# projectchrono/DEM-Engine

Hardware: AMD Instinct MI355X
Metric: clump*steps/s (higher is better)
Workload: dtype f32 physics / f64 geometry

## Files before the change

### dem-engine_amd/csrc/deme_kernels.h

```cpp
#pragma once
#include "deme_device.h"
#include "deme_owner_cols.h"

namespace deme_dev {

#define DEME_NULL_BINID_DEV 0xFFFFFFFFu
#define DEME_ST_VELOCITY 1u
#define DEME_ST_NONFINITE 2u
#define DEME_ST_INCIDENCE 4u
#define DEME_MAX_BINS_PER_SPHERE 0xFFFFFFu

struct DetectCounters {
    unsigned long long nContactsRaw;
    unsigned int nActiveBins;
    unsigned int maxInBin;
    unsigned int status;
    unsigned int pad0;
    unsigned long long nIncidence;
    unsigned int pad[8];
};

#define DEME_KEY_SEGS 64u
#define DEME_KEY_SEG_STRIDE 16u
struct DetectBlock {
    DetectCounters c;
    unsigned long long segCount[DEME_KEY_SEGS];
    unsigned long long segCtr[DEME_KEY_SEGS * DEME_KEY_SEG_STRIDE];
};
struct DetectHead {
    DetectCounters c;
    unsigned long long segCount[DEME_KEY_SEGS];
};
struct KeyArena {
    uint64_t* keys;
    unsigned long long* ctr;
    uint64_t segCap;
    uint32_t segMask;
};
__device__ inline uint32_t arena_seg(const KeyArena& a) {
    return blockIdx.x & a.segMask;
}
__device__ inline unsigned long long arena_reserve(const KeyArena& a, uint32_t seg, unsigned long long n) {
    return atomicAdd(&a.ctr[seg * DEME_KEY_SEG_STRIDE], n);
}
__device__ inline void arena_store(const KeyArena& a, uint32_t seg, unsigned long long slot, uint64_t key) {
    if (slot < a.segCap)
        a.keys[(uint64_t)seg * a.segCap + slot] = key;
}
__device__ void bin_stats_block(const uint2* __restrict__ perBlock, uint32_t nBlocks, uint32_t block, DetectCounters* ctr);
__global__ __launch_bounds__(256) void k_compact_keys(const uint64_t* __restrict__ in, uint64_t segCap, DetectBlock* blk, uint32_t xOff,
                                                      uint64_t* __restrict__ out, const uint2* __restrict__ stats, uint32_t nStats) {
    __shared__ unsigned long long sStart, sCount;
    const uint32_t seg = blockIdx.y;
    if (threadIdx.x < 64) {
        static_assert(DEME_KEY_SEGS == 64, "one lane per segment");
        const unsigned long long raw = blk->segCtr[threadIdx.x * DEME_KEY_SEG_STRIDE];
        if (stats && seg == 0 && blockIdx.x == 0)
            blk->segCount[threadIdx.x] = raw;
        const unsigned long long cnt = min(raw, (unsigned long long)segCap);
        unsigned long long inc = cnt;
        for (int d = 1; d < 64; d <<= 1) {
            const unsigned long long u = __shfl_up(inc, d);
            if ((int)threadIdx.x >= d)
                inc += u;
        }
        if (threadIdx.x == seg)
            sStart = inc - cnt, sCount = cnt;
    }
    __syncthreads();
    const uint64_t i = ((uint64_t)xOff + blockIdx.x) * blockDim.x + threadIdx.x;
    if (i < sCount)
        out[sStart + i] = in[(uint64_t)seg * segCap + i];
    if (stats && seg == 0)
        for (uint32_t b = blockIdx.x; b * 2048u < nStats; b += gridDim.x)
            bin_stats_block(stats, nStats, b, &blk->c);
}

__global__ __launch_bounds__(256) void k_margins(const DevParams p, OwnerRec* owners, uint32_t drift,
                                                 DetectCounters* ctr) {
    const uint32_t o = blockIdx.x * blockDim.x + threadIdx.x;
    if (o >= p.nOwners)
        return;
    OwnerRec* r = owners + o;
    const double vx = r->vx, vy = r->vy, vz = r->vz;
    float absv = (float)sqrt(vx * vx + vy * vy + vz * vz);
    if (!isfinite(absv))
        atomicOr(&ctr->status, DEME_ST_NONFINITE);
    else if (absv > p.errOutVel)
        atomicOr(&ctr->status, DEME_ST_VELOCITY);
    if (absv > p.approxMaxVel)
        absv = p.approxMaxVel;
    const float extra = p.familyTrivial ? 0.f : p.familyExtra[fam_of(r->family)];
    r->margin = (float)((double)(absv * p.expSafetyMulti + p.expSafetyAdder) * (double)p.h * (double)drift + (double)extra);
}

__global__ __launch_bounds__(256) void k_set_margins(uint32_t n, OwnerRec* owners, const float* m, const uint32_t* __restrict__ o2e) {
    const uint32_t o = blockIdx.x * blockDim.x + threadIdx.x;
    if (o < n)
        owners[o].margin = m[o2e ? o2e[o] : o];
}

struct ObjWorld {
    double x, y, z;
    float dx, dy, dz;
    float size1, nsign, margin;
    uint32_t type, family;
};

__global__ __launch_bounds__(256) void k_sphere_prep(const DevParams p, const OwnerRec* __restrict__ owners,
                                                     const SphereRec* __restrict__ spheres, GeoRec* __restrict__ geo,
                                                     uint4* __restrict__ binLo, uint2* __restrict__ binN,
                                                     uint32_t* __restrict__ partial, const KeyArena ar, DetectCounters* ctr,
                                                     uint16_t* __restrict__ sphFam) {
    __shared__ ObjWorld sObj[64];
    __shared__ uint32_t sWaveSum[4];
    const uint32_t s = blockIdx.x * blockDim.x + threadIdx.x;
    const bool valid = s < p.nSpheres;
    d3 pos{0, 0, 0};
    double rBin = 0;
    uint32_t fam = 0, myCount = 0;
    bool ghostOnce = false;
    if (valid) {
        const SphereRec sr = load_sphere(spheres, s);
        const OwnerRec o = load_owner(owners, sr.owner);
        const float4 c = p.comp[sr.comp];
        const d3 op = decode_pos(o.voxelID, o.locX, o.locY, o.locZ, p);
        const f3 rel = rot_apply(rot_coeffs(o.qw, o.qx, o.qy, o.qz), mk3(c.x, c.y, c.z));
        pos = {op.x + (double)rel.x, op.y + (double)rel.y, op.z + (double)rel.z};
        rBin = (double)c.w;
        rBin += o.margin;
        float rSweep = c.w;
        rSweep += o.margin;
        fam = fam_of(o.family);
        ghostOnce = ghost_of(o.family) && (p.hasGhosts & 2u);
        GeoRec g;
        g.x = pos.x, g.y = pos.y, g.z = pos.z, g.r = rSweep, g.owner = p.o2e ? p.o2e[sr.owner] : sr.owner;
        geo[s] = g;
        if (!(p.familyTrivial && !p.hasGhosts))
            sphFam[s] = (uint16_t)o.family;
        uint32_t lx, hx, ly, hy, lz, hz;
        bin_range(pos.x, rBin, p.binSize, p.nbX, lx, hx);
        bin_range(pos.y, rBin, p.binSize, p.nbY, ly, hy);
        bin_range(pos.z, rBin, p.binSize, p.nbZ, lz, hz);
        const uint32_t nx = hx - lx + 1, ny = hy - ly + 1, nz = hz - lz + 1;
        binLo[s] = make_uint4(lx, ly, lz, nx);
        binN[s] = make_uint2(ny, nz);
        const uint64_t n64 = (uint64_t)nx * ny * nz;
        if (n64 > DEME_MAX_BINS_PER_SPHERE)
            atomicOr(&ctr->status, DEME_ST_INCIDENCE);
        myCount = (n64 > DEME_MAX_BINS_PER_SPHERE) ? 0u : (uint32_t)n64;
    }
    {
        uint32_t sum = myCount;
        for (int off = 32; off > 0; off >>= 1)
            sum += (uint32_t)__shfl_xor((int)sum, off);
        if ((threadIdx.x & 63u) == 0)
            sWaveSum[threadIdx.x >> 6] = sum;
        __syncthreads();
        if (threadIdx.x == 0)
            partial[blockIdx.x] = sWaveSum[0] + sWaveSum[1] + sWaveSum[2] + sWaveSum[3];
    }

    for (uint32_t ob0 = 0; ob0 < p.nAnal; ob0 += 64) {
        __syncthreads();
        if (threadIdx.x < 64 && ob0 + threadIdx.x < p.nAnal) {
            const AnalObj ob = p.anal[ob0 + threadIdx.x];
            const OwnerRec o = load_owner(owners, ob.owner);
            const d3 op = decode_pos(o.voxelID, o.locX, o.locY, o.locZ, p);
            const RotM m = rot_coeffs(o.qw, o.qx, o.qy, o.qz);
            const f3 rp = rot_apply(m, mk3(ob.relx, ob.rely, ob.relz));
            const f3 rd = rot_apply(m, mk3(ob.rotx, ob.roty, ob.rotz));
            ObjWorld w;
            w.x = op.x + (double)rp.x, w.y = op.y + (double)rp.y, w.z = op.z + (double)rp.z;
            w.dx = rd.x, w.dy = rd.y, w.dz = rd.z;
            w.size1 = ob.size1, w.nsign = ob.normal, w.margin = o.margin;
            w.type = ob.type, w.family = fam_of(o.family);
            sObj[threadIdx.x] = w;
        }
        __syncthreads();
        {
            const uint32_t nHere = min(64u, p.nAnal - ob0);
            const uint32_t lane = threadIdx.x & 63u;
            for (uint32_t k = 0; k < nHere; k++) {
                const ObjWorld w = sObj[k];
                bool hit = valid && !ghostOnce;
                float thres = 0.f;
                if (hit && !p.familyTrivial) {
                    if (p.familyMasks[mask_pair(fam, w.family)] != 0)
                        hit = false;
                    const float ea = p.familyExtra[fam], eb = p.familyExtra[w.family];
                    thres = (ea < eb) ? ea : eb;
                }
                if (hit) {
                    d3 cp;
                    f3 nr;
                    double depth;
                    const uint32_t t = sphere_entity(pos, (float)rBin, w.type, {w.x, w.y, w.z}, mk3(w.dx, w.dy, w.dz),
                                                     w.size1, w.nsign, w.margin, cp, nr, depth);
                    hit = t && depth > (double)thres;
                }
                const unsigned long long m = __ballot(hit);
                if (m) {
                    const int leader = __ffsll((long long)m) - 1;
                    unsigned long long slot0 = 0;
                    if ((int)lane == leader)
                        slot0 = arena_reserve(ar, arena_seg(ar), (unsigned long long)__popcll(m));
                    slot0 = __shfl(slot0, leader);
                    const unsigned long long slot = slot0 + (unsigned long long)__popcll(m & ((1ull << lane) - 1ull));
                    if (hit)
                        arena_store(ar, arena_seg(ar), slot, make_key(DEME_KEY_CLASS_SA, s, ob0 + k));
                }
            }
        }
    }
}

#define DEME_SCAN_T 1024u
#define DEME_SCAN_IPT 4u
__global__ __launch_bounds__(DEME_SCAN_T) void k_scan_small(const uint32_t* in, uint32_t* out, uint32_t n, unsigned long long* totalOut) {
    __shared__ unsigned long long sWave[DEME_SCAN_T / 64];
    __shared__ unsigned long long sCarry;
    const uint32_t lane = threadIdx.x & 63u, w = threadIdx.x >> 6;
    if (threadIdx.x == 0)
        sCarry = 0;
    __syncthreads();
    for (uint32_t base = 0; base < n; base += DEME_SCAN_T * DEME_SCAN_IPT) {
        const uint32_t first = base + threadIdx.x * DEME_SCAN_IPT;
        uint32_t v[DEME_SCAN_IPT];
        unsigned long long sum = 0;
#pragma unroll
        for (uint32_t i = 0; i < DEME_SCAN_IPT; i++) {
            v[i] = first + i < n ? in[first + i] : 0u;
            sum += v[i];
        }
        unsigned long long inc = sum;
        for (int d = 1; d < 64; d <<= 1) {
            const unsigned long long u = __shfl_up(inc, d);
            if ((int)lane >= d)
                inc += u;
        }
        if (lane == 63)
            sWave[w] = inc;
        __syncthreads();
        unsigned long long run = sCarry + inc - sum, total = 0;
        for (uint32_t j = 0; j < DEME_SCAN_T / 64; j++) {
            const unsigned long long t = sWave[j];
            run += j < w ? t : 0ull;
            total += t;
        }
#pragma unroll
        for (uint32_t i = 0; i < DEME_SCAN_IPT; i++) {
            if (first + i < n)
                out[first + i] = (uint32_t)run;
            run += v[i];
        }
        __syncthreads();
        if (threadIdx.x == 0)
            sCarry += total;
        __syncthreads();
    }
    if (threadIdx.x == 0)
        *totalOut = sCarry;
}

__global__ __launch_bounds__(256) void k_fill_incidence(const DevParams p, const uint4* __restrict__ binLo,
                                                        const uint2* __restrict__ binN,
                                                        const uint32_t* __restrict__ partialPrefix,
                                                        uint32_t* __restrict__ keys, uint32_t* __restrict__ vals,
                                                        uint64_t cap) {
    __shared__ uint32_t sWaveSum[4];
    const uint32_t s = blockIdx.x * blockDim.x + threadIdx.x;
    const bool valid = s < p.nSpheres;
    const uint4 lo = valid ? binLo[s] : make_uint4(0u, 0u, 0u, 0u);
    const uint2 n = valid ? binN[s] : make_uint2(0u, 0u);
    const uint64_t n64 = (uint64_t)lo.w * n.x * n.y;
    const uint32_t cnt = n64 > DEME_MAX_BINS_PER_SPHERE ? 0u : (uint32_t)n64;
    const uint32_t lane = threadIdx.x & 63u, w = threadIdx.x >> 6;
    uint32_t inc = cnt;
    for (int d = 1; d < 64; d <<= 1) {
        const uint32_t u = (uint32_t)__shfl_up((int)inc, d);
        if ((int)lane >= d)
            inc += u;
    }
    if (lane == 63)
        sWaveSum[w] = inc;
    __syncthreads();
    uint32_t before = partialPrefix[blockIdx.x] + inc - cnt;
    for (uint32_t j = 0; j < 3; j++)
        before += j < w ? sWaveSum[j] : 0u;
    if (!cnt)
        return;
    uint64_t off = before;
    for (uint32_t k = lo.z; k < lo.z + n.y; k++)
        for (uint32_t j = lo.y; j < lo.y + n.x; j++)
            for (uint32_t i = lo.x; i < lo.x + lo.w; i++) {
                if (off < cap) {
                    keys[off] = i + j * p.nbX + k * p.nbX * p.nbY;
                    vals[off] = s;
                }
                off++;
            }
}

#ifndef SW_T
#define SW_T 256
#endif
#ifndef SW_WPB
#define SW_WPB 1
#endif
#define SW_W (2 * SW_T)
#define SW_OUT 256
#define SW_FLUSH 128

struct SweepLDS {
    float4 f[SW_W];
    uint32_t owner[SW_W], sph[SW_W], bin[SW_W];
    uint16_t fam[SW_W];
    uint32_t queue[SW_T / 64][128];
    uint64_t out[SW_OUT];
    unsigned long long gBase;
    unsigned long long headMask[SW_W / 64];
    uint32_t nOut;
    uint32_t start, endIdx, giant;
    uint32_t pop;
    uint32_t nBins, nextBin;
    uint16_t binStart[SW_W + 2];
};

__device__ inline bool pair_near(double ax, double ay, double az, float ar, uint32_t ao, double bx, double by, double bz, float br,
                                 uint32_t bo) {
    if (ao == bo)
        return false;
    const double rA = (double)ar, rB = (double)br;
    const double d2 = (ax - bx) * (ax - bx) + (ay - by) * (ay - by) + (az - bz) * (az - bz);
    return !(d2 > (rA + rB) * (rA + rB));
}

__device__ inline float sweep_radius(float x, float y, float z, float r) {
    const float mag = fabsf(x) + fabsf(y) + fabsf(z) + r;
    return (r + 0.5e-6f + 4e-7f * mag) * 1.00001f;
}
__device__ inline bool pair_near_f(float4 a, uint32_t ao, float4 b, uint32_t bo) {
    const float dx = a.x - b.x, dy = a.y - b.y, dz = a.z - b.z;
    const float rs = a.w + b.w;
    return (ao != bo) & (dx * dx + dy * dy + dz * dz <= rs * rs);
}

__device__ inline bool pair_test(const DevParams& p, double ax, double ay, double az, float ar, uint32_t ao,
                                 uint32_t af, double bx, double by, double bz, float br, uint32_t bo, uint32_t bf,
                                 uint32_t bin) {
    if (ao == bo)
        return false;
    const double rA = (double)ar, rB = (double)br;
    const double d2 = (ax - bx) * (ax - bx) + (ay - by) * (ay - by) + (az - bz) * (az - bz);
    if (d2 > (rA + rB) * (rA + rB))
        return false;
    float am = 0.f;
    if (ghost_of(af) && ghost_of(bf))
        return false;
    if ((passive_of(af) && !ghost_of(bf)) || (passive_of(bf) && !ghost_of(af)))
        return false;
    if (!p.familyTrivial) {
        af = fam_of(af), bf = fam_of(bf);
        if (p.familyMasks[mask_pair(af, bf)] != 0)
            return false;
        const float ea = p.familyExtra[af], eb = p.familyExtra[bf];
        am = (ea < eb) ? ea : eb;
    }
    d3 cp;
    f3 n;
    double depth;
    bool in = spheres_overlap(ax, ay, az, rA, bx, by, bz, rB, cp, n, depth);
    in = in && (depth > (double)am);
    return in && (point_bin(cp.x, cp.y, cp.z, p) == bin);
}

__device__ inline void sweep_emit(SweepLDS& L, bool hit, uint64_t key, uint32_t lane, const KeyArena& ar) {
    const unsigned long long m = __ballot(hit);
    if (!m)
        return;
    const int leader = __ffsll((long long)m) - 1;
    uint32_t pos0 = 0;
    if ((int)lane == leader)
        pos0 = atomicAdd(&L.nOut, (uint32_t)__popcll(m));
    pos0 = __shfl(pos0, leader);
    if (hit) {
        const uint32_t pos = pos0 + (uint32_t)__popcll(m & ((1ull << lane) - 1ull));
        if (pos < SW_OUT) {
            L.out[pos] = key;
        } else {
            arena_store(ar, arena_seg(ar), arena_reserve(ar, arena_seg(ar), 1ull), key);
        }
    }
}


__device__ inline void sweep_confirm(const DevParams& p, SweepLDS& L, const GeoRec* __restrict__ geo, const uint32_t* wq, uint32_t cnt,
                                     uint32_t lane, const KeyArena& ar) {
    __builtin_amdgcn_fence(__ATOMIC_RELEASE, "wavefront");
    __builtin_amdgcn_wave_barrier();
    __builtin_amdgcn_fence(__ATOMIC_ACQUIRE, "wavefront");
    bool hit = false;
    uint64_t key = 0;
    if (lane < cnt) {
        const uint32_t e = wq[lane];
        const uint32_t e0 = e & 0xFFFFu, e1 = e >> 16;
        uint32_t i = min(e0, e1), q = max(e0, e1);
        if (L.owner[i] > L.owner[q]) {
            const uint32_t t = i;
            i = q, q = t;
        }
        const GeoRec ga = geo[L.sph[i]], gb = geo[L.sph[q]];
        hit = pair_test(p, ga.x, ga.y, ga.z, ga.r, L.owner[i], L.fam[i], gb.x, gb.y, gb.z, gb.r, L.owner[q], L.fam[q], L.bin[q]);
        if (hit)
            key = make_key(DEME_KEY_CLASS_SS, L.sph[i], L.sph[q]);
    }
    sweep_emit(L, hit, key, lane, ar);
}

__device__ inline void sweep_flush(SweepLDS& L, uint32_t t, const KeyArena& ar) {
    const uint32_t nOut = min(L.nOut, (uint32_t)SW_OUT);
    const uint32_t seg = arena_seg(ar);
    if (t == 0)
        L.gBase = nOut ? arena_reserve(ar, seg, (unsigned long long)nOut) : 0ull;
    __syncthreads();
    for (uint32_t q = t; q < nOut; q += SW_T)
        arena_store(ar, seg, L.gBase + q, L.out[q]);
    __syncthreads();
    if (t == 0)
        L.nOut = 0;
    __syncthreads();
}

__global__ __launch_bounds__(SW_T) void k_sweep(const DevParams p, const uint32_t* __restrict__ keys,
                                                const uint32_t* __restrict__ sphIds, uint32_t P,
                                                const GeoRec* __restrict__ geo, const uint16_t* __restrict__ sphFam,
                                                const KeyArena ar, uint2* __restrict__ winStats) {
    __shared__ SweepLDS L;
    const uint32_t t = threadIdx.x;
    const uint32_t lane = t & 63u;
    const uint32_t nWin = (P + SW_T - 1) / SW_T;
    if (t == 0)
        L.nOut = 0;
    for (uint32_t win = blockIdx.x; win < nWin; win += gridDim.x) {
        const uint32_t base = win * SW_T;
        __syncthreads();
        uint32_t k0 = DEME_NULL_BINID_DEV, k1 = DEME_NULL_BINID_DEV;
        if (base + t < P)
            k0 = keys[base + t];
        if (base + SW_T + t < P)
            k1 = keys[base + SW_T + t];
        L.bin[t] = k0;
        L.bin[SW_T + t] = k1;
        if (t == 0) {
            L.start = SW_W;
            L.endIdx = SW_W;
            L.giant = 0;
            L.pop = 0;
        }
        __syncthreads();
        const uint32_t prev0 = (t == 0) ? (base == 0 ? DEME_NULL_BINID_DEV : keys[base - 1]) : L.bin[t - 1];
        const bool head0 = (base + t < P) && (k0 != prev0);
        const bool head1 = (base + SW_T + t >= P) ? (base + SW_T + t == P) : (k1 != L.bin[SW_T + t - 1]);
        if (head0)
            atomicMin(&L.start, t);
        if (head1)
            atomicMin(&L.endIdx, SW_T + t);
        if (base + t == P)
            atomicMin(&L.endIdx, t);
        __syncthreads();
        const uint32_t start = L.start;
        if (start >= SW_T) {
            if (t == 0)
                winStats[win] = make_uint2(0u, 0u);
            continue;
        }
        uint32_t end = L.endIdx;
        uint32_t giantStart = SW_W;
        if (end >= SW_W) {
            if (head0)
                atomicMax(&L.giant, t);
            __syncthreads();
            giantStart = L.giant;
            end = giantStart;
        }
        const uint32_t n_rng = end - start;
        __syncthreads();
        for (uint32_t q = t; q < n_rng; q += SW_T) {
            const uint32_t sph = sphIds[base + start + q];
            const GeoRec g = geo[sph];
            const uint32_t bq = keys[base + start + q];
            const uint32_t nbXY = p.nbX * p.nbY;
            const uint32_t iz = fast_div(bq, nbXY, p.mNbXY), rem = bq - iz * nbXY;
            const uint32_t iy = fast_div(rem, p.nbX, p.mNbX), ix = rem - iy * p.nbX;
            const float fx = (float)(g.x - (double)ix * p.binSize), fy = (float)(g.y - (double)iy * p.binSize),
                        fz = (float)(g.z - (double)iz * p.binSize);
            L.f[q] = make_float4(fx, fy, fz, sweep_radius(fx, fy, fz, g.r));
            L.owner[q] = g.owner, L.sph[q] = sph;
            L.fam[q] = (uint16_t)((p.familyTrivial && !p.hasGhosts) ? 0u : sphFam[sph]);
        }
        uint32_t b0 = DEME_NULL_BINID_DEV, b1 = DEME_NULL_BINID_DEV;
        if (t < n_rng)
            b0 = L.bin[start + t];
        if (SW_T + t < n_rng)
            b1 = L.bin[start + SW_T + t];
        __syncthreads();
        L.bin[t] = b0;
        L.bin[SW_T + t] = b1;
        __syncthreads();
        for (uint32_t q = t; q < SW_W; q += SW_T) {
            const bool head = q < n_rng && (q == 0 || L.bin[q] != L.bin[q - 1]);
            const unsigned long long hm = __ballot(head);
            if (lane == 0)
                L.headMask[q >> 6] = hm;
        }
        __syncthreads();
        for (uint32_t q = t; q < SW_W; q += SW_T) {
            const unsigned long long hm = L.headMask[q >> 6];
            if ((hm >> lane) & 1ull) {
                uint32_t idx = (uint32_t)__popcll(hm & ((1ull << lane) - 1ull));
                for (uint32_t ch = 0; ch < (q >> 6); ch++)
                    idx += (uint32_t)__popcll(L.headMask[ch]);
                L.binStart[idx] = (uint16_t)q;
            }
        }
        if (t == 0) {
            uint32_t nb = 0;
            for (uint32_t ch = 0; ch < SW_W / 64; ch++)
                nb += (uint32_t)__popcll(L.headMask[ch]);
            L.binStart[nb] = (uint16_t)n_rng;
            L.nBins = nb;
            L.nextBin = 0;
        }
        __syncthreads();
        uint32_t* wq = L.queue[t >> 6];
        uint32_t qn = 0;
        uint32_t popMine = 0;
        const uint32_t nBinsHere = L.nBins;
        auto enqueue = [&](bool near, uint32_t packed) {
            const unsigned long long nm = __ballot(near);
            if (nm) {
                if (near)
                    wq[qn + (uint32_t)__popcll(nm & ((1ull << lane) - 1ull))] = packed;
                qn += (uint32_t)__popcll(nm);
                if (qn >= 64u) {
                    sweep_confirm(p, L, geo, wq, 64u, lane, ar);
                    const uint32_t rest = qn - 64u;
                    uint32_t carry = 0;
                    if (lane < rest)
                        carry = wq[64u + lane];
                    __builtin_amdgcn_fence(__ATOMIC_RELEASE, "wavefront");
                    __builtin_amdgcn_wave_barrier();
                    if (lane < rest)
                        wq[lane] = carry;
                    qn = rest;
                }
            }
        };
        for (;;) {
            uint32_t b = 0;
            if (lane == 0)
                b = atomicAdd(&L.nextBin, 1u);
            b = (uint32_t)__builtin_amdgcn_readfirstlane((int)b);
            if (b >= nBinsHere)
                break;
            const uint32_t s = (uint32_t)__builtin_amdgcn_readfirstlane((int)L.binStart[b]);
            const uint32_t n = (uint32_t)__builtin_amdgcn_readfirstlane((int)L.binStart[b + 1]) - s;
            popMine = max(popMine, n);
            if (n < 2u)
                continue;
            const uint32_t total = n * (n - 1u) / 2u;
            const float rn = __builtin_amdgcn_rcpf((float)n);
            uint32_t m = (uint32_t)(((float)lane + 0.5f) * rn);
            uint32_t k = lane - m * n;
            m += 1u;
            const uint32_t c2 = (uint32_t)(64.5f * rn), c1 = 64u - c2 * n;
            for (uint32_t f = lane, f0 = 0; f0 < total; f0 += 64u, f += 64u) {
                const bool act = f < total;
                uint32_t j = k + m;
                j = min(j, j - n);
                const uint32_t ia = s + k, ib = act ? s + j : s + k;
                const float4 fa = L.f[ia], fb = L.f[ib];
                const uint32_t oa = L.owner[ia], ob = L.owner[ib];
                enqueue(act & pair_near_f(fa, oa, fb, ob), ia | (ib << 16));
                k += c1, m += c2;
                if (k >= n)
                    k -= n, m += 1u;
            }
        }
        if (qn) {
            sweep_confirm(p, L, geo, wq, qn, lane, ar);
            qn = 0;
        }
        if (lane == 0 && popMine)
            atomicMax(&L.pop, popMine);
        uint32_t giantPop = 0;
        if (giantStart < SW_W) {
            const uint32_t gs = base + giantStart;
            const uint32_t gbin = keys[gs];
            uint32_t lo = gs + 1, hi = P;
            while (lo < hi) {
                const uint32_t mid = lo + ((hi - lo) >> 1);
                if (keys[mid] <= gbin)
                    lo = mid + 1;
                else
                    hi = mid;
            }
            const uint32_t ge = lo;
            giantPop = ge - gs;
            for (uint32_t ta = gs; ta < ge; ta += SW_T) {
                __syncthreads();
                const uint32_t na = min((uint32_t)SW_T, ge - ta);
                if (t < na) {
                    const uint32_t sph = sphIds[ta + t];
                    const GeoRec g = geo[sph];
                    L.owner[t] = g.owner, L.sph[t] = sph;
                    L.fam[t] = (uint16_t)((p.familyTrivial && !p.hasGhosts) ? 0u : sphFam[sph]);
                }
                __syncthreads();
                for (uint32_t tb = ta; tb < ge; tb += SW_T) {
                    const uint32_t jb = tb + t;
                    const bool valid = jb < ge;
                    double mx = 0, my = 0, mz = 0;
                    float mr = 0;
                    uint32_t mo = 0, mf = 0, ms = 0;
                    if (valid) {
                        ms = sphIds[jb];
                        const GeoRec g = geo[ms];
                        mx = g.x, my = g.y, mz = g.z, mr = g.r, mo = g.owner;
                        mf = (p.familyTrivial && !p.hasGhosts) ? 0u : sphFam[ms];
                    }
                    for (uint32_t i = 0; i < na; i++) {
                        const bool act = valid && (ta + i < jb);
                        bool hit = false;
                        uint64_t key = 0;
                        if (act) {
                            const GeoRec ga = geo[L.sph[i]];
                            const bool entryFirst = L.owner[i] <= mo;
                            const double ax = entryFirst ? ga.x : mx, ay = entryFirst ? ga.y : my, az = entryFirst ? ga.z : mz;
                            const double bx = entryFirst ? mx : ga.x, by = entryFirst ? my : ga.y, bz = entryFirst ? mz : ga.z;
                            const float ar_ = entryFirst ? ga.r : mr, br_ = entryFirst ? mr : ga.r;
                            const uint32_t ao = entryFirst ? L.owner[i] : mo, bo = entryFirst ? mo : L.owner[i];
                            const uint32_t af = entryFirst ? (uint32_t)L.fam[i] : mf, bf = entryFirst ? mf : (uint32_t)L.fam[i];
                            hit = pair_test(p, ax, ay, az, ar_, ao, af, bx, by, bz, br_, bo, bf, gbin);
                            if (hit)
                                key = entryFirst ? make_key(DEME_KEY_CLASS_SS, L.sph[i], ms) : make_key(DEME_KEY_CLASS_SS, ms, L.sph[i]);
                        }
                        sweep_emit(L, hit, key, lane, ar);
                    }
                    __syncthreads();
                    if (L.nOut >= SW_FLUSH)
                        sweep_flush(L, t, ar);
                }
            }
        }
        __syncthreads();
        if (t == 0) {
            uint32_t heads = (giantStart < SW_W) ? 1u : 0u;
            for (uint32_t ch = 0; ch < SW_W / 64; ch++)
                heads += (uint32_t)__popcll(L.headMask[ch]);
            winStats[win] = make_uint2(heads, max(L.pop, giantPop));
        }
        if (L.nOut >= SW_FLUSH)
            sweep_flush(L, t, ar);
    }
    __syncthreads();
    sweep_flush(L, t, ar);
}

__device__ void bin_stats_block(const uint2* __restrict__ perBlock, uint32_t nBlocks, uint32_t block, DetectCounters* ctr) {
    __shared__ uint32_t sHeads[4], sPop[4];
    uint32_t heads = 0, pop = 0;
    {
        const uint32_t i0 = block * 2048u;
        uint2 v[8];
#pragma unroll
        for (uint32_t k = 0; k < 8; k++) {
            const uint32_t i = i0 + k * 256u + threadIdx.x;
            v[k] = (i < nBlocks) ? perBlock[i] : make_uint2(0u, 0u);
        }
#pragma unroll
        for (uint32_t k = 0; k < 8; k++) {
            heads += v[k].x;
            pop = max(pop, v[k].y);
        }
    }
    for (int off = 32; off > 0; off >>= 1) {
        heads += (uint32_t)__shfl_xor((int)heads, off);
        pop = max(pop, (uint32_t)__shfl_xor((int)pop, off));
    }
    if ((threadIdx.x & 63u) == 0) {
        sHeads[threadIdx.x >> 6] = heads;
        sPop[threadIdx.x >> 6] = pop;
    }
    __syncthreads();
    if (threadIdx.x == 0) {
        atomicAdd(&ctr->nActiveBins, sHeads[0] + sHeads[1] + sHeads[2] + sHeads[3]);
        const uint32_t m = max(max(sPop[0], sPop[1]), max(sPop[2], sPop[3]));
        if (m > 1)
            atomicMax(&ctr->maxInBin, m);
    }
    __syncthreads();
}
__global__ __launch_bounds__(256) void k_bin_stats_final(const uint2* __restrict__ perBlock, uint32_t nBlocks, DetectCounters* ctr) {
    bin_stats_block(perBlock, nBlocks, blockIdx.x, ctr);
}

__global__ __launch_bounds__(256) void k_segment_rank_sort(uint32_t n, const uint64_t* __restrict__ in, uint64_t* __restrict__ out) {
    const uint32_t i = blockIdx.x * blockDim.x + threadIdx.x;
    if (i >= n)
        return;
    const uint64_t k = in[i], seg = k >> 31;
    uint32_t s = i, rank = 0;
    while (s > 0) {
        const uint64_t q = in[s - 1];
        if ((q >> 31) != seg)
            break;
        rank += (q <= k) ? 1u : 0u;
        s--;
    }
    for (uint32_t j = i + 1; j < n; j++) {
        const uint64_t q = in[j];
        if ((q >> 31) != seg)
            break;
        rank += (q < k) ? 1u : 0u;
    }
    out[s + rank] = k;
}

__global__ __launch_bounds__(256) void k_history(uint32_t nNew, const uint64_t* __restrict__ newKeys, uint32_t nPrev,
                                                 const uint64_t* __restrict__ prevKeys, uint32_t* __restrict__ mapping,
                                                 uint32_t* __restrict__ zeroA, uint32_t nZeroA, uint32_t* __restrict__ zeroB,
                                                 uint32_t nZeroB) {
    const uint32_t c = blockIdx.x * blockDim.x + threadIdx.x;
    for (uint32_t i = c; i < nZeroA; i += gridDim.x * blockDim.x)
        zeroA[i] = 0u;
    for (uint32_t i = c; i < nZeroB; i += gridDim.x * blockDim.x)
        zeroB[i] = 0u;
    if (c >= nNew)
        return;
    const uint64_t k = newKeys[c];
    uint32_t lo = 0, hi = nPrev;
    if (nPrev) {
        uint32_t g = (uint32_t)(((uint64_t)c * nPrev) / nNew);
        g = min(g, nPrev - 1);
        if (prevKeys[g] < k) {
            lo = g + 1;
            uint32_t step = 8;
            while (lo < nPrev) {
                const uint32_t j = (lo + step < nPrev) ? lo + step : nPrev - 1;
                if (prevKeys[j] < k) {
                    lo = j + 1;
                    step <<= 2;
                } else {
                    hi = j;
                    break;
                }
            }
        } else {
            hi = g;
            uint32_t step = 8;
            while (hi > 0) {
                const uint32_t j = (hi > step) ? hi - step : 0;
                if (prevKeys[j] < k) {
                    lo = j + 1;
                    break;
                }
                hi = j;
                step <<= 2;
            }
        }
    }
    while (lo < hi) {
        const uint32_t mid = lo + ((hi - lo) >> 1);
        if (prevKeys[mid] < k)
            lo = mid + 1;
        else
            hi = mid;
    }
    mapping[c] = (lo < nPrev && prevKeys[lo] == k) ? lo : 0xFFFFFFFFu;
}

__global__ __launch_bounds__(256) void k_migrate(uint32_t nNew, uint32_t nW, const uint32_t* __restrict__ mapping,
                                                 uint32_t nPrevStored, const float* __restrict__ oldW,
                                                 float* __restrict__ newW) {
    const uint32_t c = blockIdx.x * blockDim.x + threadIdx.x;
    if (c >= nNew)
        return;
    const uint32_t m = mapping[c];
    const bool have = (m != 0xFFFFFFFFu) && (m < nPrevStored);
    if (nW == 4) {
        float4 v = make_float4(0, 0, 0, 0);
        if (have)
            v = reinterpret_cast<const float4*>(oldW)[m];
        reinterpret_cast<float4*>(newW)[c] = v;
    } else {
        for (uint32_t w = 0; w < nW; w++)
            newW[(size_t)c * nW + w] = have ? oldW[(size_t)m * nW + w] : 0.f;
    }
}

struct GatherArgs {
    const uint32_t* aStart;
    const uint32_t* bStart;
    const uint32_t* bIdx;
    const uint8_t* heavy;
    const float4* conA4;
    const float2* conA2;
    const float4* conB4;
    const float2* conB2;
    const float4* aSum;
    const AccRec* nextAcc;
    uint32_t world;
    uint32_t tile;
    const float4* rec32;
    const uint32_t* revSlot;
    const float4* revAcc;
    uint32_t revPhase;
    uint32_t revInIntegrator;
};

__device__ inline void gather_b_load(const GatherArgs& g, uint32_t idx, float4& c4, float2& c2) {
    if (g.tile) {
        const float2* r24 = reinterpret_cast<const float2*>(g.rec32) + 3 * (size_t)idx;
        const float2 r0 = r24[0], r1 = r24[1];
        c4 = make_float4(r0.x, r0.y, r1.x, r1.y), c2 = r24[2];
    } else {
        conb_load(g.conB4, g.conB2, idx, c4, c2);
    }
}

__device__ inline void acc_from_world(const DevParams& p, const OwnerRec& r, float4& a, float4& al) {
    const float4 mp = p.massProps[r.inertiaOff];
    const RotM R = rot_coeffs(r.qw, r.qx, r.qy, r.qz);
    const f3 tl = rot_apply(rot_transpose(R), mk3(al.x, al.y, al.z));
    a = make_float4(a.x / mp.x, a.y / mp.x, a.z / mp.x, 0.f);
    al = make_float4(tl.x / mp.y, tl.y / mp.z, tl.z / mp.w, 0.f);
}


__device__ inline void a_side_sum(const GatherArgs& g, uint32_t o, uint32_t s, uint32_t e, float& ax, float& ay, float& az,
                                  float& lx, float& ly, float& lz) {
    if (g.tile) {
        const float2* t24 = reinterpret_cast<const float2*>(g.aSum) + 3 * (size_t)o;
        const float2 u = t24[0], v = t24[1], w = t24[2];
        ax = u.x, ay = u.y, az = v.x, lx = v.y, ly = w.x, lz = w.y;
        return;
    }
    if (a_run_in_one_block(s, e)) {
        const float4 v = g.aSum[2 * (size_t)o], w = g.aSum[2 * (size_t)o + 1];
        ax = v.x, ay = v.y, az = v.z, lx = w.x, ly = w.y, lz = w.z;
        return;
    }
    for (uint32_t ia = s; ia < e; ia += 4) {
        float4 c4[4];
        float2 c2[4];
#pragma unroll
        for (int k = 0; k < 4; k++) {
            const bool ok = ia + k < e;
            c4[k] = ok ? g.conA4[ia + k] : make_float4(0, 0, 0, 0);
            c2[k] = ok ? g.conA2[ia + k] : make_float2(0, 0);
        }
#pragma unroll
        for (int k = 0; k < 4; k++)
            if (ia + k < e) {
                ax += c4[k].x, ay += c4[k].y, az += c4[k].z;
                lx += c4[k].w, ly += c2[k].x, lz += c2[k].y;
            }
    }
}

__device__ inline void gather_owner(const GatherArgs& g, uint32_t o, float4& a, float4& al) {
    float ax = 0.f, ay = 0.f, az = 0.f, lx = 0.f, ly = 0.f, lz = 0.f;
    const uint32_t ib0 = g.bStart[o], eb = g.bStart[o + 1];
    a_side_sum(g, o, g.aStart[o], g.aStart[o + 1], ax, ay, az, lx, ly, lz);
    for (uint32_t ib = ib0; ib < eb; ib += 4) {
        uint32_t idx[4];
        float4 c4[4];
        float2 c2[4];
#pragma unroll
        for (int k = 0; k < 4; k++)
            idx[k] = (ib + k < eb) ? g.bIdx[ib + k] : 0u;
#pragma unroll
        for (int k = 0; k < 4; k++) {
            const bool ok = ib + k < eb;
            c4[k] = make_float4(0, 0, 0, 0);
            c2[k] = make_float2(0, 0);
            if (ok)
                gather_b_load(g, idx[k], c4[k], c2[k]);
        }
// ... 735 lines not shown
```

Baseline: 6.475 billion.

## Pair two partners per slot in bin sweep with byte-offset LDS indexing

Restructures the in-bin all-pairs sweep so each lane evaluates two partner spheres per iteration, sharing the load of the first sphere. The pair enumeration moves into a new helper header that works on byte-scaled indices, and the packed queue entries now hold byte offsets that are shifted back down in the confirm step. The enqueue builds its mask from three separate ballots and uses mbcnt to find each lane's slot, and the per-bin loop constants are kept in scalar registers. This is meant to cut per-pair index arithmetic and LDS loads, but the byte-offset indexing and the odd/even slot validity limits are subtle and could miss or duplicate pairs.

```diff
diff --git a/dem-engine_amd/csrc/deme_kernels.h b/dem-engine_amd/csrc/deme_kernels.h
--- a/dem-engine_amd/csrc/deme_kernels.h
+++ b/dem-engine_amd/csrc/deme_kernels.h
@@ -1,6 +1,7 @@
 #pragma once
 #include "deme_device.h"
 #include "deme_owner_cols.h"
+#include "deme_sweep_pairing.h"
 
 namespace deme_dev {
 
@@ -340,10 +341,13 @@
     const float mag = fabsf(x) + fabsf(y) + fabsf(z) + r;
     return (r + 0.5e-6f + 4e-7f * mag) * 1.00001f;
 }
-__device__ inline bool pair_near_f(float4 a, uint32_t ao, float4 b, uint32_t bo) {
+__device__ inline bool pair_dist_f(float4 a, float4 b) {
     const float dx = a.x - b.x, dy = a.y - b.y, dz = a.z - b.z;
     const float rs = a.w + b.w;
-    return (ao != bo) & (dx * dx + dy * dy + dz * dz <= rs * rs);
+    return dx * dx + dy * dy + dz * dz <= rs * rs;
+}
+__device__ inline bool pair_near_f(float4 a, uint32_t ao, float4 b, uint32_t bo) {
+    return (ao != bo) & pair_dist_f(a, b);
 }
 
 __device__ inline bool pair_test(const DevParams& p, double ax, double ay, double az, float ar, uint32_t ao,
@@ -404,7 +408,7 @@
     uint64_t key = 0;
     if (lane < cnt) {
         const uint32_t e = wq[lane];
-        const uint32_t e0 = e & 0xFFFFu, e1 = e >> 16;
+        const uint32_t e0 = (e & 0xFFFFu) >> 2, e1 = e >> 18;
         uint32_t i = min(e0, e1), q = max(e0, e1);
         if (L.owner[i] > L.owner[q]) {
             const uint32_t t = i;
@@ -533,30 +537,31 @@
             L.nextBin = 0;
         }
         __syncthreads();
-        uint32_t* wq = L.queue[t >> 6];
+        uint32_t* wq = L.queue[__builtin_amdgcn_readfirstlane((int)(t >> 6))];
         uint32_t qn = 0;
         uint32_t popMine = 0;
         const uint32_t nBinsHere = L.nBins;
-        auto enqueue = [&](bool near, uint32_t packed) {
-            const unsigned long long nm = __ballot(near);
-            if (nm) {
-                if (near)
-                    wq[qn + (uint32_t)__popcll(nm & ((1ull << lane) - 1ull))] = packed;
-                qn += (uint32_t)__popcll(nm);
-                if (qn >= 64u) {
-                    sweep_confirm(p, L, geo, wq, 64u, lane, ar);
-                    const uint32_t rest = qn - 64u;
-                    uint32_t carry = 0;
-                    if (lane < rest)
-                        carry = wq[64u + lane];
-                    __builtin_amdgcn_fence(__ATOMIC_RELEASE, "wavefront");
-                    __builtin_amdgcn_wave_barrier();
-                    if (lane < rest)
-                        wq[lane] = carry;
-                    qn = rest;
-                }
+        auto enqueue = [&](bool exists, bool otherOwner, bool near, uint32_t packed) {
+            const unsigned long long nm =
+                __builtin_amdgcn_ballot_w64(exists) & __builtin_amdgcn_ballot_w64(otherOwner) & __builtin_amdgcn_ballot_w64(near);
+            if (exists & otherOwner & near)
+                (wq + qn)[__builtin_amdgcn_mbcnt_hi((uint32_t)(nm >> 32), __builtin_amdgcn_mbcnt_lo((uint32_t)nm, 0u))] = packed;
+            qn += (uint32_t)__popcll(nm);
+            if (qn >= 64u) {
+                sweep_confirm(p, L, geo, wq, 64u, lane, ar);
+                const uint32_t rest = qn - 64u;
+                uint32_t carry = 0;
+                if (lane < rest)
+                    carry = wq[64u + lane];
+                __builtin_amdgcn_fence(__ATOMIC_RELEASE, "wavefront");
+                __builtin_amdgcn_wave_barrier();
+                if (lane < rest)
+                    wq[lane] = carry;
+                qn = rest;
             }
         };
+        const char* const ldsF = reinterpret_cast<const char*>(L.f);
+        const char* const ldsOwner = reinterpret_cast<const char*>(L.owner);
         for (;;) {
             uint32_t b = 0;
             if (lane == 0)
@@ -569,23 +574,22 @@
             popMine = max(popMine, n);
             if (n < 2u)
                 continue;
-            const uint32_t total = n * (n - 1u) / 2u;
             const float rn = __builtin_amdgcn_rcpf((float)n);
-            uint32_t m = (uint32_t)(((float)lane + 0.5f) * rn);
-            uint32_t k = lane - m * n;
-            m += 1u;
-            const uint32_t c2 = (uint32_t)(64.5f * rn), c1 = 64u - c2 * n;
-            for (uint32_t f = lane, f0 = 0; f0 < total; f0 += 64u, f += 64u) {
-                const bool act = f < total;
-                uint32_t j = k + m;
-                j = min(j, j - n);
-                const uint32_t ia = s + k, ib = act ? s + j : s + k;
-                const float4 fa = L.f[ia], fb = L.f[ib];
-                const uint32_t oa = L.owner[ia], ob = L.owner[ib];
-                enqueue(act & pair_near_f(fa, oa, fb, ob), ia | (ib << 16));
-                k += c1, m += c2;
-                if (k >= n)
-                    k -= n, m += 1u;
+            SweepBin<4> sb = sweep_bin<4>(s, n, (uint32_t)__builtin_amdgcn_readfirstlane((int)sweep_div(64u, rn)));
+            sb.c1U = (uint32_t)__builtin_amdgcn_readfirstlane((int)sb.c1U);
+            asm("" : "+s"(sb.c1U));
+            SweepSlot sl = sweep_slot(sb, n, lane, 0u, rn);
+            for (uint32_t g0 = 0; g0 < sb.slots; g0 += 64u) {
+                const SweepPartners pr = sweep_partners(sb, sl);
+                const float4 fa = *reinterpret_cast<const float4*>(ldsF + (sl.kU << 2));
+                const uint32_t oa = *reinterpret_cast<const uint32_t*>(ldsOwner + sl.kU);
+                const float4 fb1 = *reinterpret_cast<const float4*>(ldsF + (pr.j1U << 2));
+                const uint32_t ob1 = *reinterpret_cast<const uint32_t*>(ldsOwner + pr.j1U);
+                const float4 fb2 = *reinterpret_cast<const float4*>(ldsF + (pr.j2U << 2));
+                const uint32_t ob2 = *reinterpret_cast<const uint32_t*>(ldsOwner + pr.j2U);
+                enqueue(pr.v1, oa != ob1, pair_dist_f(fa, fb1), sl.kU | (pr.j1U << 16));
+                enqueue(pr.v2, oa != ob2, pair_dist_f(fa, fb2), sl.kU | (pr.j2U << 16));
+                sweep_next(sb, sl);
             }
         }
         if (qn) {
diff --git a/dem-engine_amd/csrc/deme_sweep_pairing.h b/dem-engine_amd/csrc/deme_sweep_pairing.h
--- /dev/null
+++ b/dem-engine_amd/csrc/deme_sweep_pairing.h
@@ -0,0 +1,86 @@
+#pragma once
+#include <cstdint>
+
+#if defined(__HIPCC__) || defined(__CUDACC__)
+#define DEME_PAIRING_HD __host__ __device__
+#else
+#define DEME_PAIRING_HD
+#endif
+#if defined(__HIP_DEVICE_COMPILE__)
+#define DEME_PAIRING_MUL24(a, b) __umul24((a), (b))
+#else
+#define DEME_PAIRING_MUL24(a, b) ((a) * (b))
+#endif
+
+namespace deme_dev {
+
+template <uint32_t U>
+struct SweepBin {
+    uint32_t base, nU, endU;
+    uint32_t pLast;
+    uint32_t slots;
+    uint32_t c1U, c2;
+    uint32_t lim1;
+    int32_t lim2;
+};
+
+struct SweepSlot {
+    uint32_t kU;
+    uint32_t p;
+};
+
+struct SweepPartners {
+    uint32_t j1U, j2U;
+    bool v1, v2;
+};
+
+DEME_PAIRING_HD inline uint32_t sweep_div(uint32_t x, float rn) {
+    return (uint32_t)(((float)x + 0.5f) * rn);
+}
+
+template <uint32_t U>
+DEME_PAIRING_HD inline SweepBin<U> sweep_bin(uint32_t first, uint32_t n, uint32_t c2) {
+    SweepBin<U> b;
+    b.base = U * first, b.nU = U * n, b.endU = b.base + b.nU;
+    b.pLast = ((n >> 1) - 1u) >> 1;
+    b.slots = (b.pLast + 1u) * n;
+    b.c2 = c2;
+    b.c1U = U * 64u - DEME_PAIRING_MUL24(c2, b.nU);
+    b.lim1 = U * (n * (n - 1u) / 2u) + b.base;
+    b.lim2 = (int32_t)b.lim1 - (int32_t)b.nU;
+    return b;
+}
+
+template <uint32_t U>
+DEME_PAIRING_HD inline SweepSlot sweep_slot(const SweepBin<U>& b, uint32_t n, uint32_t lane, uint32_t trip, float rn) {
+    const uint32_t g = lane + 64u * trip;
+    SweepSlot s;
+    s.p = sweep_div(g, rn);
+    s.kU = b.base + U * (g - DEME_PAIRING_MUL24(s.p, n));
+    return s;
+}
+
+template <uint32_t U>
+DEME_PAIRING_HD inline void sweep_next(const SweepBin<U>& b, SweepSlot& s) {
+    s.kU += b.c1U;
+    const bool wrap = s.kU >= b.endU;
+    s.kU = wrap ? s.kU - b.nU : s.kU;
+    s.p += b.c2 + (wrap ? 1u : 0u);
+}
+
+template <uint32_t U>
+DEME_PAIRING_HD inline SweepPartners sweep_partners(const SweepBin<U>& b, const SweepSlot& s) {
+    SweepPartners r;
+    const uint32_t pc = s.p < b.pLast ? s.p : b.pLast;
+    uint32_t j0 = s.kU + (2u * U) * pc;
+    j0 = j0 >= b.endU - U ? j0 - b.nU : j0;
+    const uint32_t j1 = j0 + U;
+    const uint32_t j2 = j0 == b.endU - 2u * U ? b.base : j0 + 2u * U;
+    r.j1U = j1, r.j2U = j2;
+    const uint32_t f = DEME_PAIRING_MUL24(s.p, 2u * b.nU) + s.kU;
+    r.v1 = f < b.lim1;
+    r.v2 = (int32_t)f < b.lim2;
+    return r;
+}
+
+}
```

Result: no change. 6.518 billion (median of 6 runs) (+0.7%).
